# dbolya/yolact

Hardware: AMD Instinct MI355X
Metric: images/sec (550x550, batch 8 per GPU), YOLACT yolact_resnet50 forward + Detect (Fast NMS) (higher is better)
Workload: dtype f32 (fp32 in / fp32 accumulate / fp32 out; 92 % of the GEMM time on fp16x2 tiles = every fp32 operand as two fp16 pieces by round to nearest (22 significant bits + 2 signs: exact for ~2/3 of all fp32 values, one fp32 ulp otherwise), 3 exact piece products per product on the fp16 matrix pipe; measure

## Files before the change

### include/yolact_amd.h

```cpp
#ifndef YOLACT_AMD_H
#define YOLACT_AMD_H
#include <stddef.h>
#include <stdint.h>

#ifdef __cplusplus
extern "C" {
#endif

#define YMI_ABI_VERSION 9

#define YMI_EFORMAT (-4)
#define YMI_EUNSUPPORTED (-5)

enum { YMI_ACT_NONE = 0, YMI_ACT_RELU = 1, YMI_ACT_LEAKY01 = 2, YMI_ACT_TANH = 3, YMI_ACT_SIGMOID = 4 };
enum { YMI_RES_NONE = 0, YMI_RES_ADD = 1, YMI_RES_BILINEAR = 2 };

typedef struct {
  int32_t n0, n1;
  int32_t act;
  int32_t row_stride;
  int64_t batch_stride;
  float *ptr;
} ymi_conv_seg;

// ... 468 lines not shown
  const float *x;
  float *y;
  int32_t B, H, W, cout_pad;
  const void *w_h2;
  const float *scale_h2, *bias;
  float *y_amax;
  int32_t kpad, _pad0;
} ymi_stem_desc;
int ymi_stem_pool_f32(const ymi_stem_desc *d, void *stream);

typedef struct ymi_chain_desc {
  const float *x, *res;
  float *y, *z;
  const void *w_a_h2, *w_b_h2;
  const float *scale_a_h2, *bias_a, *scale_b_h2, *bias_b;
  const float *x_amax;
  float *y_amax, *z_amax;
  int64_t M;
  int32_t ldx, res_ld, ldy, ldz;
  int32_t k_a, n_a, n_b;
  int32_t cout_pad_a, cout_pad_b;
  int32_t act_a, act_b, _pad0;
  const float *res_amax;
  float gain_a, bias_max_a;
} ymi_chain_desc;
int ymi_pointwise_chain_f32(const ymi_chain_desc *d, void *stream);

typedef struct ymi_stage_exit_desc {
  ymi_chain_desc chain;
  int32_t B, H, W, y_stride;
} ymi_stage_exit_desc;
int ymi_stage_exit_chain_f32(const ymi_stage_exit_desc *d, void *stream);

enum { YMI_OP_NOP = 0, YMI_OP_CONV = 1, YMI_OP_WINO = 2, YMI_OP_DCN = 3, YMI_OP_CHAIN = 4, YMI_OP_STEM = 5, YMI_OP_INPUT = 6,
       YMI_OP_BILINEAR = 7, YMI_OP_MAXPOOL = 8, YMI_OP_BILINEAR_ADD = 9, YMI_OP_RECORD = 10, YMI_OP_WAIT = 11, YMI_OP_MEMSET = 12,
       YMI_OP_STAGE_EXIT = 13 };
enum { YMI_SEC_NONE = 0, YMI_SEC_BACKBONE = 1, YMI_SEC_FPN = 2, YMI_SEC_PROTO = 3, YMI_SEC_HEADS = 4 };
typedef struct ymi_plan_op {
  int32_t kind;
  int32_t stream;
  int32_t section;
  int32_t _pad;
  const void *desc;
  void *p[3];
  int64_t i[8];
  double f[2];
} ymi_plan_op;
int ymi_event_create(void **ev);
int ymi_event_destroy(void *ev);
int ymi_plan_run(const ymi_plan_op *ops, int first, int last, void *stream_a, void *stream_b, void *const *events, int overlap,
                 int skip_sections, int32_t *failed_op);

enum {
  YMI_WS_WINO_V = 1,
  YMI_WS_WINO_M = 2,
  YMI_WS_SPLITK = 3,
  YMI_WS_MASK_IOU = 4,
  YMI_WS_JPEG_COEFS = 5,
  YMI_WS_JPEG_PLANES = 6,
  YMI_WS_DETECT_SCORES_T = 7,
  YMI_WS_DETECT_PER_PRIOR = 8,
  YMI_WS_DETECT_CAND = 9,
  YMI_WS_DETECT_REC = 10,
  YMI_WS_AMAX_SLOT = 11,
  YMI_WS_RLE_COUNTS = 12,
  YMI_WS_DETECT_GREEDY = 13,
  YMI_WS_JPEG_ENC = 14,
  YMI_WS_JPEG_ENC_OUT = 15,
  YMI_WS_MASK_LOSS = 16,
// ... 31 lines not shown
```

### yolact_amd/_lib.py

```python
from __future__ import annotations

import ctypes as C
import os

_HERE = os.path.dirname(os.path.abspath(__file__))
LIB_PATH = os.path.join(_HERE, 'libyolact_amd.so')

ABI_VERSION = 9

ACT_NONE, ACT_RELU, ACT_LEAKY01, ACT_TANH, ACT_SIGMOID = 0, 1, 2, 3, 4
RES_NONE, RES_ADD, RES_BILINEAR = 0, 1, 2
TILE_AUTO, TILE_128x128, TILE_128x64, TILE_64x64, TILE_128x32, TILE_64x128 = 0, 1, 2, 3, 4, 5
TILE_32x32_K4, TILE_64x32_K2, TILE_32x64_K2 = 6, 7, 8
TILE_64x64_S3, TILE_64x64_S4, TILE_64x128_S3, TILE_128x64_S3, TILE_32x32_K4_S4, TILE_64x32_K2_S3, TILE_32x64_K2_S3 = range(9, 16)
TILE_NAMES = {1: '128x128', 2: '128x64', 3: '64x64', 4: '128x32', 5: '64x128', 6: '32x32k4', 7: '64x32k2', 8: '32x64k2',
              9: '64x64s3', 10: '64x64s4', 11: '64x128s3', 12: '128x64s3', 13: '32x32k4s4', 14: '64x32k2s3', 15: '32x64k2s3',
              16: '128x128w8', 17: '256x128w8', 18: '128x256w8', 19: '128x128s3', 20: '128x128w8s3', 21: '256x128w8s3',
              22: '128x128w8s4'}
TILE_128x128_W8, TILE_256x128_W8, TILE_128x256_W8 = 16, 17, 18
TILE_128x128_S3, TILE_128x128_W8_S3, TILE_256x128_W8_S3, TILE_128x128_W8_S4 = 19, 20, 21, 22
TILE_WG_128x256 = 23
TILE_X3 = 32
X3_BASE_TILES = (1, 2, 3, 5, 6, 7, 8, 9, 11, 12, 16, 17, 19, 20, 21, 22)
for _t in X3_BASE_TILES:
# ... 188 lines not shown


JPEG_SUB_444, JPEG_SUB_420 = 0, 2
JPEG_HEADER_BYTES = 623


class ChainDesc(C.Structure):
    _fields_ = [('x', C.c_void_p), ('res', C.c_void_p), ('y', C.c_void_p), ('z', C.c_void_p),
                ('w_a_h2', C.c_void_p), ('w_b_h2', C.c_void_p),
                ('scale_a_h2', C.c_void_p), ('bias_a', C.c_void_p), ('scale_b_h2', C.c_void_p), ('bias_b', C.c_void_p),
                ('x_amax', C.c_void_p), ('y_amax', C.c_void_p), ('z_amax', C.c_void_p),
                ('M', C.c_int64), ('ldx', C.c_int32), ('res_ld', C.c_int32), ('ldy', C.c_int32), ('ldz', C.c_int32),
                ('k_a', C.c_int32), ('n_a', C.c_int32), ('n_b', C.c_int32), ('cout_pad_a', C.c_int32), ('cout_pad_b', C.c_int32),
                ('act_a', C.c_int32), ('act_b', C.c_int32), ('_pad0', C.c_int32),
                ('res_amax', C.c_void_p), ('gain_a', C.c_float), ('bias_max_a', C.c_float)]


class StageExitDesc(C.Structure):
    _fields_ = [('chain', ChainDesc), ('B', C.c_int32), ('H', C.c_int32), ('W', C.c_int32), ('y_stride', C.c_int32)]


class StemDesc(C.Structure):
    _fields_ = [('x', C.c_void_p), ('y', C.c_void_p), ('B', C.c_int32), ('H', C.c_int32), ('W', C.c_int32), ('cout_pad', C.c_int32),
                ('w_h2', C.c_void_p), ('scale_h2', C.c_void_p), ('bias', C.c_void_p), ('y_amax', C.c_void_p),
                ('kpad', C.c_int32), ('_pad0', C.c_int32)]


class PlanOp(C.Structure):
    _fields_ = [('kind', C.c_int32), ('stream', C.c_int32), ('section', C.c_int32), ('_pad', C.c_int32), ('desc', C.c_void_p),
                ('p', C.c_void_p * 3), ('i', C.c_int64 * 8), ('f', C.c_double * 2)]


(OP_NOP, OP_CONV, OP_WINO, OP_DCN, OP_CHAIN, OP_STEM, OP_INPUT, OP_BILINEAR, OP_MAXPOOL, OP_BILINEAR_ADD, OP_RECORD, OP_WAIT,
 OP_MEMSET, OP_STAGE_EXIT) = range(14)
SEC_NONE, SEC_BACKBONE, SEC_FPN, SEC_PROTO, SEC_HEADS = range(5)


class MaskIouShape(C.Structure):
    _fields_ = [('A', C.c_int32), ('B', C.c_int32), ('n', C.c_int64)]


class ApMatchDesc(C.Structure):
    _fields_ = [('cls', C.c_void_p), ('box_score', C.c_void_p), ('mask_score', C.c_void_p), ('box_iou', C.c_void_p),
                ('mask_iou', C.c_void_p), ('crowd_box_iou', C.c_void_p), ('crowd_mask_iou', C.c_void_p), ('gt_cls', C.c_void_p),
                ('crowd_cls', C.c_void_p), ('rec_key', C.c_void_p), ('rec_score', C.c_void_p), ('rec_flags', C.c_void_p),
                ('gt_count', C.c_void_p), ('base', C.c_int64), ('cap', C.c_int64),
                ('N', C.c_int32), ('G', C.c_int32), ('Gc', C.c_int32), ('num_classes', C.c_int32)]


class ApFinalizeDesc(C.Structure):
    _fields_ = [('sorted_key', C.c_void_p), ('perm', C.c_void_p), ('rec_flags', C.c_void_p), ('gt_count', C.c_void_p),
                ('ap', C.c_void_p), ('empty', C.c_void_p), ('M', C.c_int64), ('cap', C.c_int64),
                ('num_classes', C.c_int32), ('_pad0', C.c_int32)]


AP_NUM_THRESH, AP_MAX_DET, AP_MAX_GT = 10, 1024, 2048


class RleShape(C.Structure):
    _fields_ = [('N', C.c_int32), ('h', C.c_int32), ('w', C.c_int32), ('cap', C.c_int32)]


(WS_WINO_V, WS_WINO_M, WS_SPLITK, WS_MASK_IOU, WS_JPEG_COEFS, WS_JPEG_PLANES, WS_DETECT_SCORES_T, WS_DETECT_PER_PRIOR,
 WS_DETECT_CAND, WS_DETECT_REC, WS_AMAX_SLOT, WS_RLE_COUNTS, WS_DETECT_GREEDY, WS_JPEG_ENC, WS_JPEG_ENC_OUT,
 WS_MASK_LOSS, WS_MATCH, WS_BOX_LOSS, WS_CLASS_LOSS, WS_SEGM_LOSS, WS_MASKIOU_INPUT, WS_CONV_BWD, WS_MASKIOU_HEAD,
 WS_CONV_WGRAD, WS_BN, WS_STEM_WGRAD) = range(1, 27)

# ... 29 lines not shown
    ('ymi_dcn_v2_forward_f32', C.c_int, [C.POINTER(DcnDesc), _P]),
    ('ymi_dcn_v2_backward_f32', C.c_int, [C.POINTER(DcnBwdDesc), _P]),
    ('ymi_mask_loss_f32', C.c_int, [C.POINTER(MaskLossDesc), _P]),
    ('ymi_match_f32', C.c_int, [C.POINTER(MatchDesc), _P]),
    ('ymi_box_loss_f32', C.c_int, [_P, _P, _P, _I, _I, _F, _P, _P, _P, _P]),
    ('ymi_class_loss_f32', C.c_int, [C.POINTER(ClassLossDesc), _P]),
    ('ymi_segm_loss_f32', C.c_int, [C.POINTER(SegmLossDesc), _P]),
    ('ymi_maskiou_input_f32', C.c_int, [C.POINTER(MaskIouInputDesc), _P]),
    ('ymi_maskiou_input_bwd_f32', C.c_int, [C.POINTER(MaskIouInputDesc), _P]),
    ('ymi_conv2d_bwd_nhwc_f32', C.c_int, [C.POINTER(ConvBwdDesc), _P]),
    ('ymi_global_maxpool_bwd_nhwc_f32', C.c_int, [_P, _P, _P, _I, _I, _I, _P]),
    ('ymi_maskiou_head_f32', C.c_int, [C.POINTER(MaskIouHeadDesc), _P]),
    ('ymi_act_bwd_f32', C.c_int, [_P, _P, _P, C.c_long] + [_I] * 6 + [_P]),
    ('ymi_conv_wgrad_nhwc_f32', C.c_int, [C.POINTER(ConvWgradDesc), _P]),
    ('ymi_conv_dgrad_s2_nhwc_f32', C.c_int, [C.POINTER(ConvDgradDesc), _P]),
    ('ymi_bn_fwd_nhwc_f32', C.c_int, [C.POINTER(BnDesc), _P]),
    ('ymi_bn_bwd_nhwc_f32', C.c_int, [C.POINTER(BnDesc), _P]),
    ('ymi_stem_wgrad_nhwc_f32', C.c_int, [C.POINTER(StemWgradDesc), _P]),
    ('ymi_maxpool_fwd_nhwc_f32', C.c_int, [_P, _P, _I, _I, _I, _I, _P]),
    ('ymi_maxpool_bwd_nhwc_f32', C.c_int, [_P, _P, _P, _I, _I, _I, _I, _P]),
    ('ymi_bilinear_bwd_nhwc_f32', C.c_int, [_P, _P, _P] + [_I] * 7 + [_P]),
    ('ymi_bilinear_size_bwd_nhwc_f32', C.c_int, [_P, _P] + [_I] * 6 + [_P]),
    ('ymi_composite_masks_u8', C.c_int, [_P, _P, _P, _I, _I, _I, _F, _P, _P]),
    ('ymi_mask_iou_f32', C.c_int, [_P, _P, _I, _I, C.c_long, _I, _P, _P, _P]),
    ('ymi_jaccard_f32', C.c_int, [_P, _P, _I, _I, _I, _P, _P]),
    ('ymi_mask_bits_f32', C.c_int, [_P, _I, C.c_long, _P, _P]),
    ('ymi_mask_upsample_bits', C.c_int, [_P, _I, _I, _I, _I, _I, _F, _P, _P]),
    ('ymi_mask_iou_bits', C.c_int, [_P, _P, _I, _I, C.c_long, _I, _P, _P]),
    ('ymi_ap_match_f32', C.c_int, [C.POINTER(ApMatchDesc), _P]),
    ('ymi_ap_finalize_f64', C.c_int, [C.POINTER(ApFinalizeDesc), _P]),
    ('ymi_stem_pool_f32', C.c_int, [_P, _P]),
    ('ymi_pointwise_chain_f32', C.c_int, [_P, _P]),
    ('ymi_stage_exit_chain_f32', C.c_int, [_P, _P]),
    ('ymi_mask_rle_f32', C.c_int, [_P, _I, _I, _I, _P, _P, _I, _P]),
    ('ymi_mask_rle_upsampled_f32', C.c_int, [_P, _I, _I, _I, _I, _I, _F, _P, _P, _I, _P]),
    ('ymi_rle_to_string', C.c_int, [_P, _P, _I, _I, _P, _P, _I, _P]),
    ('ymi_fast_base_transform_f32', C.c_int, [_P, _P, _I, _I, _I, _I, _I, C.POINTER(C.c_float), C.POINTER(C.c_float), _I, _I, _P]),
    ('ymi_jpeg_parse', C.c_int, [_P, C.c_size_t, C.POINTER(JpegInfo)]),
    ('ymi_jpeg_decode_coefs', C.c_int, [_P, C.c_size_t, _P, C.c_int64, _P, C.POINTER(JpegInfo)]),
    ('ymi_jpeg_reconstruct_bgr_u8', C.c_int, [C.POINTER(JpegInfo), _P, _P, _P, _P, _P]),
    ('ymi_jpeg_write_header', C.c_int, [_I, _I, _I, _I, _P, C.c_size_t, C.POINTER(C.c_size_t)]),
    ('ymi_jpeg_enc_qtables', C.c_int, [_I, _P]),
    ('ymi_jpeg_encode_bgr_u8', C.c_int, [C.POINTER(JpegEncDesc), _P]),
    ('ymi_coco_poly_fill_u8', C.c_int, [_P, _I, _I, _I, _P]),
    ('ymi_coco_rle_fill_u8', C.c_int, [_P, C.c_long, _I, _I, _P]),
    ('ymi_coco_rle_string_fill_u8', C.c_int, [C.c_char_p, C.c_long, _I, _I, _P]),
    ('ymi_event_create', C.c_int, [C.POINTER(C.c_void_p)]),
    ('ymi_event_destroy', C.c_int, [_P]),
    ('ymi_plan_run', C.c_int, [C.POINTER(PlanOp), _I, _I, _P, _P, C.POINTER(C.c_void_p), _I, _I, C.POINTER(C.c_int32)]),
    ('ymi_workspace_bytes', C.c_int64, [_I, _P]),
    ('ymi_calib_mfma_f16', C.c_int, [_P, _I, _I, C.POINTER(C.c_double), _P]),
    ('ymi_calib_hbm_copy', C.c_int, [_P, _P, C.c_long, C.POINTER(C.c_double), _P]),
    ('ymi_calib_l2_read', C.c_int, [_P, C.c_long, _I, _I, _P, C.POINTER(C.c_double), _P]),
    ('ymi_calib_latency', C.c_int, [_P, C.c_long, _I, _I, _P, _P]),
    ('ymi_debug_set_trace', C.c_int, [_P, C.c_long]),
    ('ymi_prof_enable', C.c_int, [_I]),
    ('ymi_prof_count', C.c_int, []),
    ('ymi_prof_read', C.c_int, [_I, C.POINTER(C.c_float), C.POINTER(C.c_double), C.POINTER(C.c_int32),
                                C.POINTER(C.c_int32)]),
    ('ymi_prof_reset', C.c_int, []),
]

_lib = None


def lib():
# ... 33 lines not shown
```

### yolact_amd/csrc/api.cpp

```cpp
#include "../../include/yolact_amd.h"
#include <hip/hip_runtime_api.h>

extern "C" {

int64_t ymi_detect_greedy_layout(const ymi_detect_desc *d, int64_t off[4]);
int64_t ymi_jpeg_enc_layout(int h, int w, int sub, int64_t off[8], int64_t *out_bound);
int64_t ymi_mask_loss_ws_bytes(const ymi_mask_loss_desc *d);
int64_t ymi_match_ws_bytes(const ymi_match_desc *d);
int64_t ymi_box_loss_ws_bytes(const ymi_match_desc *d);
int64_t ymi_class_loss_ws_bytes(const ymi_class_loss_desc *d);
int64_t ymi_segm_loss_ws_bytes(const ymi_segm_loss_desc *d);
int64_t ymi_maskiou_input_ws_bytes(const ymi_maskiou_input_desc *d);
int64_t ymi_conv_bwd_ws_bytes(const ymi_conv_bwd_desc *d);
int64_t ymi_maskiou_head_ws_bytes(const ymi_maskiou_head_desc *d);
int64_t ymi_conv_wgrad_ws_bytes(const ymi_conv_wgrad_desc *d);
int64_t ymi_bn_ws_bytes(const ymi_bn_desc *d);
int64_t ymi_stem_wgrad_ws_bytes(const ymi_stem_wgrad_desc *d);

int ymi_abi_version(void) { return YMI_ABI_VERSION; }

const char *ymi_strerror(int code) {
  switch (code) {
    case 0: return "ok";
    case -1: return "bad argument / unsupported configuration";
    case -2: return "shape or alignment constraint violated";
    case -3: return "null pointer";
    case YMI_EFORMAT: return "corrupt or truncated input stream";
    case YMI_EUNSUPPORTED: return "valid input outside the supported subset";
  }
  if (code > 0) return hipGetErrorString((hipError_t)code);
  return "unknown error";
}

int64_t ymi_workspace_bytes(int what, const void *desc) {
  auto cdiv = [](int64_t a, int64_t b) { return (a + b - 1) / b; };
  if (what == YMI_WS_AMAX_SLOT) return (int64_t)YMI_AMAX_SUB * YMI_AMAX_STRIDE * 4;
  if (!desc) return -3;
  switch (what) {
    case YMI_WS_WINO_V:
    case YMI_WS_WINO_M: {
      const ymi_wino_desc *d = (const ymi_wino_desc *)desc;
      const int m = d->m == 4 ? 4 : 2;
      if ((d->m != 0 && d->m != 2 && d->m != 4) || d->B < 1 || d->H < 1 || d->W < 1 || d->C < 1 || d->Cout < 1) return -1;
      const int64_t G = (int64_t)(m + 2) * (m + 2), T = (int64_t)d->B * cdiv(d->H, m) * cdiv(d->W, m);
      return 4 * G * T * (what == YMI_WS_WINO_V ? (int64_t)d->C : cdiv(d->Cout, 4) * 4);
    }
    case YMI_WS_SPLITK: {
      const ymi_conv_desc *d = (const ymi_conv_desc *)desc;
      if (d->B < 1 || d->Ho < 1 || d->Wo < 1 || d->Cout < 1 || d->split_k < 0) return -1;
      return d->split_k > 1 ? 4 * (int64_t)d->split_k * d->B * d->Ho * d->Wo * d->Cout : 0;
    }
    case YMI_WS_MASK_IOU: {
// ... 54 lines not shown
```

### yolact_amd/csrc/plan_exec.cpp

```cpp
#include "../../include/yolact_amd.h"
#include <hip/hip_runtime_api.h>

extern "C" {

int ymi_event_create(void **ev) {
  if (!ev) return -3;
  hipEvent_t e;
  const hipError_t rc = hipEventCreateWithFlags(&e, hipEventDisableTiming);
  if (rc != hipSuccess) return (int)rc;
  *ev = (void *)e;
  return 0;
}

int ymi_event_destroy(void *ev) {
  if (!ev) return -3;
  return (int)hipEventDestroy((hipEvent_t)ev);
}

int ymi_plan_run(const ymi_plan_op *ops, int first, int last, void *stream_a, void *stream_b, void *const *events, int overlap,
                 int skip_sections, int32_t *failed_op) {
  if (!ops || first < 0 || last < first) return -1;
  void *const sb = overlap ? stream_b : stream_a;
  for (int k = first; k < last; ++k) {
    const ymi_plan_op &o = ops[k];
    if (o.section && (skip_sections & (1 << o.section))) continue;
    void *const s = o.stream == 1 ? sb : stream_a;
    int rc = 0;
    switch (o.kind) {
      case YMI_OP_NOP: break;
      case YMI_OP_CONV: rc = ymi_conv2d_nhwc_f32((const ymi_conv_desc *)o.desc, s); break;
      case YMI_OP_WINO: rc = ymi_conv3x3_winograd_f32((const ymi_wino_desc *)o.desc, s); break;
      case YMI_OP_DCN: rc = ymi_dcn_v2_forward_f32((const ymi_dcn_desc *)o.desc, s); break;
      case YMI_OP_CHAIN: rc = ymi_pointwise_chain_f32((const ymi_chain_desc *)o.desc, s); break;
      case YMI_OP_STAGE_EXIT: rc = ymi_stage_exit_chain_f32((const ymi_stage_exit_desc *)o.desc, s); break;
      case YMI_OP_STEM: rc = ymi_stem_pool_f32((const ymi_stem_desc *)o.desc, s); break;
      case YMI_OP_INPUT:
        rc = o.p[2] ? ymi_nchw_to_nhwc4_amax_f32((const float *)o.p[0], (float *)o.p[1], (int)o.i[0], (int)o.i[1], (int)o.i[2], (int)o.i[3],
                                                 (float *)o.p[2], s)
                    : ymi_nchw_to_nhwc4_f32((const float *)o.p[0], (float *)o.p[1], (int)o.i[0], (int)o.i[1], (int)o.i[2], (int)o.i[3], s);
        break;
      case YMI_OP_BILINEAR:
        rc = ymi_bilinear_nhwc_f32((const float *)o.p[0], (float *)o.p[1], (int)o.i[0], (int)o.i[1], (int)o.i[2], (int)o.i[3], (int)o.i[4],
                                   (int)o.i[5], (float)o.f[0], (float)o.f[1], (int)o.i[6], s);
        break;
      case YMI_OP_MAXPOOL:
        rc = ymi_maxpool3x3s2_nhwc_f32((const float *)o.p[0], (float *)o.p[1], (int)o.i[0], (int)o.i[1], (int)o.i[2], (int)o.i[3],
                                       (int)o.i[4], (int)o.i[5], s);
        break;
      case YMI_OP_BILINEAR_ADD:
        rc = ymi_bilinear_add_nhwc_f32((const float *)o.p[0], (float *)o.p[1], (int)o.i[0], (int)o.i[1], (int)o.i[2], (int)o.i[3],
                                       (int)o.i[4], (int)o.i[5], (float *)o.p[2], s);
        break;
      case YMI_OP_RECORD:
        if (overlap) rc = (int)hipEventRecord((hipEvent_t)events[o.i[0]], (hipStream_t)s);
        break;
      case YMI_OP_WAIT:
        if (overlap) rc = (int)hipStreamWaitEvent((hipStream_t)s, (hipEvent_t)events[o.i[0]], 0);
        break;
      case YMI_OP_MEMSET:
        rc = (int)hipMemsetAsync(o.p[0], 0, (size_t)o.i[0], (hipStream_t)s);
        break;
      default: rc = -1;
    }
    if (rc != 0) {
      if (failed_op) *failed_op = k;
      return rc;
    }
// ... 6 lines not shown
```

### yolact_amd/engine.py

```python
from __future__ import annotations

import ctypes as C
import json
import os
from typing import List, Optional

import torch
import torch.nn as nn

from . import _lib as L
from .config import act_name, make_priors_host
from . import modules as M


def _ceil(a, b):
    return (a + b - 1) // b * b


SPLIT_DEFAULT = '2'
TUNE_GEN = 5
AMAX_SLOT_FLOATS = 16 * 64
TUNE_DIR = os.path.join(os.path.dirname(os.path.abspath(__file__)), 'tune')
_table_cache = {}

# ... 1074 lines not shown
        if timer is not None and not all(hasattr(timer, a) for a in ('start', 'stop', 'env')):
            timer = None
        if timer is None and self.native_exec:
            nat = self._native_plan()
            if nat is not None:
                det = self._run_native(nat, x, sa, sb, two, detect, skip_proto)
                self.mark_done()
                return proto, det
        if self.h2:
            self.amax[:self._nslots * AMAX_SLOT_FLOATS].zero_()
        self._sec = None
        try:
            det = self._dispatch(x, cur, sa, sb, two, detect, timer, skip_proto)
        finally:
            if timer is not None and self._sec is not None:
                timer.stop(self._sec)
        self.mark_done()
        return proto, det

    _SEC_ID = {'backbone': L.SEC_BACKBONE, 'fpn': L.SEC_FPN, 'proto': L.SEC_PROTO, 'pred_heads': L.SEC_HEADS}

    def _native_plan(self):
        key = (self.ops.version, len(self.ops)) if isinstance(self.ops, _OpList) else tuple(map(id, self.ops))
        if self._native is not None and self._native[0] == key:
            return self._native[1]
        lib = self.lib
        n = len(self.ops)
        arr = (L.PlanOp * (n + 1))()
        arr[0].kind, arr[0].stream = L.OP_MEMSET, 0
        arr[0].p[0], arr[0].i[0] = self.amax.data_ptr(), 4 * self._nslots * AMAX_SLOT_FLOATS
        ev_index, det_idx, in_idx, ok = {}, None, None, True
        by_fn = {id(lib.ymi_conv2d_nhwc_f32): L.OP_CONV, id(lib.ymi_conv3x3_winograd_f32): L.OP_WINO,
                 id(lib.ymi_dcn_v2_forward_f32): L.OP_DCN, id(lib.ymi_pointwise_chain_f32): L.OP_CHAIN,
                 id(lib.ymi_stage_exit_chain_f32): L.OP_STAGE_EXIT}
        for k, (fn, args, name, where) in enumerate(self.ops):
            o = arr[k + 1]
            o.stream = 1 if where == 'B' else 0
            o.section = self._SEC_ID.get(self.sections[k], 0) if self.sections[k] else 0
            if fn == 'input':
                a = self.in_args
                o.kind, in_idx = L.OP_INPUT, k + 1
                o.p[1] = a[1]
                o.p[2] = self.in_amax[2] if self.h2 else None
                o.i[0], o.i[1], o.i[2], o.i[3] = a[2], a[3], a[4], a[5]
            elif fn == 'stem':
                o.kind, o.desc = L.OP_STEM, C.addressof(args)
            elif fn == 'nop':
                o.kind = L.OP_NOP
            elif fn in ('record', 'wait'):
                o.kind = L.OP_RECORD if fn == 'record' else L.OP_WAIT
                o.i[0] = ev_index.setdefault(args, len(ev_index))
            elif fn == 'detect':
                o.kind, det_idx = L.OP_NOP, k + 1
            elif id(fn) in by_fn:
                o.kind, o.desc = by_fn[id(fn)], C.addressof(args.contents)
            elif fn is lib.ymi_bilinear_nhwc_f32:
                o.kind = L.OP_BILINEAR
                o.p[0], o.p[1] = args[0], args[1]
                for q in range(6):
                    o.i[q] = args[2 + q]
                o.f[0], o.f[1], o.i[6] = args[8].value, args[9].value, args[10]
            elif fn is lib.ymi_maxpool3x3s2_nhwc_f32:
                o.kind = L.OP_MAXPOOL
                o.p[0], o.p[1] = args[0], args[1]
                for q in range(6):
                    o.i[q] = args[2 + q]
            elif fn is lib.ymi_bilinear_add_nhwc_f32:
# ... 69 lines not shown
                a = self.in_args
                if self.h2:
                    rc = lib.ymi_nchw_to_nhwc4_amax_f32(x.data_ptr(), a[1], a[2], a[3], a[4], a[5], self.in_amax[2], s)
                else:
                    rc = lib.ymi_nchw_to_nhwc4_f32(x.data_ptr(), a[1], a[2], a[3], a[4], a[5], s)
            elif fn == 'nop' or (skip_proto and nsec == 'proto'):
                continue
            elif fn == 'stem':
                args.x = x.data_ptr()
                rc = lib.ymi_stem_pool_f32(C.byref(args), s)
            elif fn == 'record':
                if two:
                    self.events[args].record(self.stream_b if where == 'B' else cur)
                continue
            elif fn == 'wait':
                if two:
                    (self.stream_b if where == 'B' else cur).wait_event(self.events[args])
                continue
            elif fn == 'detect':
                if detect is not None:
                    det = detect(s)
                continue
            elif isinstance(args, tuple):
                rc = fn(*args, s)
            else:
                rc = fn(args, s)
            if rc != 0:
                L.check(rc, name)
        return det

    def tune(self, x: torch.Tensor, reps: int = 3):
        mode = os.environ.get('YOLACT_AMD_AUTOTUNE', '1')
        self.tune_table, self.wino_table, self.tune_misses = [], [], 0
        if mode == '0':
            return []
        cache_path = os.environ.get('YOLACT_AMD_TUNE_CACHE')
        disk = {}
        if mode != 'force':
            disk.update(load_tune_table(self.device))
            if cache_path and os.path.exists(cache_path):
                disk.update(_read_table_file(cache_path))
        n0 = len(disk)
        self.run(x)
        s = L.stream_ptr()
        e0, e1 = torch.cuda.Event(enable_timing=True), torch.cuda.Event(enable_timing=True)
        measure = mode != 'table'
        self._tune_direct(e0, e1, s, reps, disk, measure)
        self._tune_winograd(e0, e1, s, reps, disk, measure)
        self._fuse_pointwise_chains(e0, e1, s, reps, disk, measure)
        torch.cuda.synchronize(self.device)
        if cache_path and (len(disk) != n0 or mode == 'force'):
            _write_table_file(cache_path, disk, self.device)
        self.tune_entries = disk
        return self.tune_table

    autotune = tune

    def _splitk_ws(self, where, numel):
        ws = self._sk_ws.get(where)
        if ws is None or ws.numel() < numel:
            ws = self._sk_ws[where] = torch.empty(numel, dtype=torch.float32, device=self.device)
            for fn, dptr, _n, w in self.ops:
                if fn is self.lib.ymi_conv2d_nhwc_f32 and w == where and dptr.contents.split_k > 1:
                    dptr.contents.split_ws = ws.data_ptr()
                elif fn is self.lib.ymi_dcn_v2_forward_f32 and w == where and dptr.contents.conv.split_k > 1:
                    dptr.contents.conv.split_ws = ws.data_ptr()
        return ws

    @staticmethod
    def _splitk_ok(d):
        return (d.kh == 1 and d.kw == 1 and d.pad == 0 and d.Cin == d.Kpad and d.Cin % 32 == 0 and d.nseg == 1
                and d.Cout % 4 == 0 and d.seg[0].act <= L.ACT_LEAKY01 and d.res_mode in (L.RES_NONE, L.RES_ADD)
                and d.B * d.Ho * d.Wo <= 16384 and d.Kpad >= 256)

    def _fuse_pointwise_chains(self, e0, e1, s, reps, disk, measure):
        self.chain_table, self.chainx_table = [], []
        if not self.h2 or os.environ.get('YOLACT_AMD_CHAIN', '1') != '1':
            return
        lib = self.lib

        def timed(run):
            run()
# ... 168 lines not shown
            if overlap(zs, span(cd.y, cd.ldy)) or overlap(zs, span(cd.x, cd.ldx)) or (cd.res and overlap(zs, span(cd.res, cd.res_ld))):
                continue
            xptr = C.pointer(xd)
            name = n3 + '+' + n1
            shape = str((d3.B, d3.Ho, d3.Wo)) + self.mode_key
            ent = disk.get('chainx' + shape)
            if mode == 'force':
                ent = [1, 0.0, 0.0]
            if ent is None:
                self.tune_misses += 1
                if not measure or lib.ymi_stage_exit_chain_f32(xptr, s) != 0:
                    continue
                run3 = lambda: f3(p3, s)
                c1 = disk.get('chain1' + shape)
                if c1 is not None and c1[0]:
                    cc = L.ChainDesc.from_buffer_copy(cd)
                    cc.z, cc.w_b_h2, cc.scale_b_h2, cc.bias_b, cc.z_amax, cc.n_b = None, None, None, None, None, 64
                    ccp = C.pointer(cc)
                    if lib.ymi_pointwise_chain_f32(ccp, s) == 0:
                        run3 = lambda: lib.ymi_pointwise_chain_f32(ccp, s)
                t_plan = timed(lambda: (run3(), f1(p1, s)))
                t_one = timed(lambda: lib.ymi_stage_exit_chain_f32(xptr, s))
                ent = disk['chainx' + shape] = [1 if t_one < 0.97 * t_plan else 0, round(t_plan, 4), round(t_one, 4)]
            self.chainx_table.append((name, ent[0], ent[1], ent[2]))
            if ent[0] and lib.ymi_stage_exit_chain_f32(xptr, s) == 0:
                self.keepalive.append(xd)
                self.ops[i3] = (lib.ymi_stage_exit_chain_f32, xptr, name, w3)
                self.ops[i1] = ('nop', None, n1 + '[fused into ' + n3 + ']', w1)
                names = [n for n, _ in self.conv_meta]
                if n3 in names and n1 in names:
                    a, b = names.index(n3), names.index(n1)
                    if b > a + 1:
                        self.conv_meta.insert(a + 1, self.conv_meta.pop(b))

    def _apply_choice(self, fn, dptr, where, val, s):
        d = dptr.contents.conv if fn is self.lib.ymi_dcn_v2_forward_f32 else dptr.contents
        tile, S = int(val) & 255, int(val) >> 8
        d.tile = tile
        if S > 1:
            is_dcn = fn is self.lib.ymi_dcn_v2_forward_f32
            if tile & L.TILE_DCNP:
                nk_ = d.Kpad // 32
                if -(-nk_ // S) * (S - 1) >= nk_:
                    return -1
            elif is_dcn or not self._splitk_ok(d) or (d.Kpad // 32) % S:
                return -1
            d.split_k = S
            d.split_ws = self._splitk_ws(where, S * d.B * d.Ho * d.Wo * d.Cout).data_ptr()
        else:
            d.split_k = 0
        return fn(dptr, s)

    @staticmethod
    def _pipe_ok(d):
        return ((d.kh, d.kw, d.pad) in ((3, 3, 1), (1, 1, 0)) and d.Cin % 32 == 0 and d.Kpad == d.kh * d.kw * d.Cin and d.Kpad >= 64
                and d.nseg == 1 and d.Cout % 4 == 0 and d.seg[0].n0 == 0 and d.seg[0].act <= L.ACT_LEAKY01
                and d.seg[0].row_stride % 4 == 0 and d.seg[0].batch_stride == d.Ho * d.Wo * d.seg[0].row_stride
                and d.res_mode in (L.RES_NONE, L.RES_ADD))

    @staticmethod
    def dcnp_candidates(d, dcn=False):
        M, nk = d.B * d.Ho * d.Wo, d.Kpad // 32
        out = []
        for t, name in sorted(L.DCNP_TILES.items()):
            bm, bn = (int(v) for v in name[4:].split('w')[0].split('x'))
            if (bn > 128 and d.Cout < 256) or (dcn and t in L.DCNP_PLAIN_ONLY) or (bn == 32) != (d.Cout <= 32):
# ... 274 lines not shown
```

Baseline: 2362.

## Add specialized persistent kernel for 1x1 expand convs with autotuned install

Adds a dedicated persistent HIP kernel for 1x1 stride-1 expansion convolutions (Cin 128/256, Cout = 4*Cin). Each block keeps its 256-wide weight slice in registers, streams activation rows through a register ring, and splits them to fp16 hi/lo pieces in LDS for the three-product MFMA scheme, with a fused scale/bias/activation/residual epilogue. The kernel is timed against the existing conv path during autotuning and installed only when it wins by a margin. This adds a new kernel, a plan op kind and tuning-cache entries, and relies on grid sizing by CU count and on specific shape constraints.

```diff
diff --git a/include/yolact_amd.h b/include/yolact_amd.h
--- a/include/yolact_amd.h
+++ b/include/yolact_amd.h
@@ -524,9 +524,11 @@
 } ymi_stage_exit_desc;
 int ymi_stage_exit_chain_f32(const ymi_stage_exit_desc *d, void *stream);
 
+int ymi_conv1x1_expand_f32(const ymi_conv_desc *d, void *stream);
+
 enum { YMI_OP_NOP = 0, YMI_OP_CONV = 1, YMI_OP_WINO = 2, YMI_OP_DCN = 3, YMI_OP_CHAIN = 4, YMI_OP_STEM = 5, YMI_OP_INPUT = 6,
        YMI_OP_BILINEAR = 7, YMI_OP_MAXPOOL = 8, YMI_OP_BILINEAR_ADD = 9, YMI_OP_RECORD = 10, YMI_OP_WAIT = 11, YMI_OP_MEMSET = 12,
-       YMI_OP_STAGE_EXIT = 13 };
+       YMI_OP_STAGE_EXIT = 13, YMI_OP_EXPAND = 14 };
 enum { YMI_SEC_NONE = 0, YMI_SEC_BACKBONE = 1, YMI_SEC_FPN = 2, YMI_SEC_PROTO = 3, YMI_SEC_HEADS = 4 };
 typedef struct ymi_plan_op {
   int32_t kind;
diff --git a/yolact_amd/_lib.py b/yolact_amd/_lib.py
--- a/yolact_amd/_lib.py
+++ b/yolact_amd/_lib.py
@@ -244,7 +244,7 @@
 
 
 (OP_NOP, OP_CONV, OP_WINO, OP_DCN, OP_CHAIN, OP_STEM, OP_INPUT, OP_BILINEAR, OP_MAXPOOL, OP_BILINEAR_ADD, OP_RECORD, OP_WAIT,
- OP_MEMSET, OP_STAGE_EXIT) = range(14)
+ OP_MEMSET, OP_STAGE_EXIT, OP_EXPAND) = range(15)
 SEC_NONE, SEC_BACKBONE, SEC_FPN, SEC_PROTO, SEC_HEADS = range(5)
 
 
@@ -340,6 +340,7 @@
     ('ymi_stem_pool_f32', C.c_int, [_P, _P]),
     ('ymi_pointwise_chain_f32', C.c_int, [_P, _P]),
     ('ymi_stage_exit_chain_f32', C.c_int, [_P, _P]),
+    ('ymi_conv1x1_expand_f32', C.c_int, [C.POINTER(ConvDesc), _P]),
     ('ymi_mask_rle_f32', C.c_int, [_P, _I, _I, _I, _P, _P, _I, _P]),
     ('ymi_mask_rle_upsampled_f32', C.c_int, [_P, _I, _I, _I, _I, _I, _F, _P, _P, _I, _P]),
     ('ymi_rle_to_string', C.c_int, [_P, _P, _I, _I, _P, _P, _I, _P]),
diff --git a/yolact_amd/csrc/api.cpp b/yolact_amd/csrc/api.cpp
--- a/yolact_amd/csrc/api.cpp
+++ b/yolact_amd/csrc/api.cpp
@@ -1,5 +1,7 @@
 #include "../../include/yolact_amd.h"
 #include <hip/hip_runtime_api.h>
+
+int ymi_internal_expand_conv(const ymi_conv_desc *d, hipStream_t s);
 
 extern "C" {
 
@@ -18,6 +20,11 @@
 int64_t ymi_stem_wgrad_ws_bytes(const ymi_stem_wgrad_desc *d);
 
 int ymi_abi_version(void) { return YMI_ABI_VERSION; }
+
+int ymi_conv1x1_expand_f32(const ymi_conv_desc *d, void *stream) {
+  if (!d) return -3;
+  return ymi_internal_expand_conv(d, (hipStream_t)stream);
+}
 
 const char *ymi_strerror(int code) {
   switch (code) {
diff --git a/yolact_amd/csrc/expand.hip b/yolact_amd/csrc/expand.hip
--- /dev/null
+++ b/yolact_amd/csrc/expand.hip
@@ -0,0 +1,258 @@
+#include "gemm_h2.h"
+#include <stdlib.h>
+#include <type_traits>
+
+int ymi_internal_prof_begin(double flops, int tile, int kind, hipStream_t s);
+void ymi_internal_prof_end(int idx, hipStream_t s);
+
+namespace {
+
+using namespace ymi_h2;
+
+typedef unsigned u32x4 __attribute__((ext_vector_type(4)));
+
+constexpr int BM = 64, BN = 256, NWAVE = 8, NT = 64 * NWAVE;
+constexpr int A_BYTES = 2 * BM * 64, B_BYTES = 2 * BN * 64;
+constexpr int NSA = 3, NSU = 3;
+constexpr int JT = BM / 32, NU = 4 * JT;
+constexpr int RA = BM / (NT / 8);
+constexpr int OFF_SC = NSA * A_BYTES, OFF_BI = OFF_SC + BN * 4, OFF_U = OFF_BI + BN * 4, EX_LDS = OFF_U + NSU * B_BYTES;
+constexpr int UPC = (2 * BN / 16) / NWAVE;
+static_assert(UPC == 4 && RA == 1 && JT == 2 && EX_LDS <= 160 * 1024, "block shape");
+#define EX_PIN() __builtin_amdgcn_sched_barrier(0)
+#define EX_MFMA(a, b, c) __builtin_amdgcn_mfma_f32_32x32x16_f16(a, b, c, 0, 0, 0)
+
+struct ExParams {
+  const float *x, *scale_h2, *bias, *x_amax, *res;
+  const void *w_h2;
+  float *y, *y_amax;
+  int M, ldx, Cout, cout_pad, ldy, res_ld, res_after_act, act;
+  int tiles_n, bpc, groups;
+  unsigned w_plane;
+};
+
+template <int NK>
+__global__ __launch_bounds__(NT) void expand_us_k(const ExParams p) {
+#if defined(__HIP_DEVICE_COMPILE__)
+  __shared__ __attribute__((aligned(16))) char lds[EX_LDS];
+  const int t = threadIdx.x, lane = t & 63, wave = __builtin_amdgcn_readfirstlane(t >> 6);
+  const int lr = lane & 31, hh = lane >> 5;
+  const int lb = ymi_xcd_remap((int)blockIdx.x, (int)gridDim.x);
+  const int tn = lb / p.bpc, jb = lb % p.bpc;
+  const int row0 = 32 * (int)(((long)jb * p.groups) / p.bpc);
+  int rend = 32 * (int)(((long)(jb + 1) * p.groups) / p.bpc);
+  rend = rend < p.M ? rend : p.M;
+  const int ntile = (rend - row0 + BM - 1) / BM;
+
+  const bool has_res = p.res != nullptr;
+  const __amdgpu_buffer_rsrc_t xrs = buf_rsrc(p.x, rend * p.ldx * 4);
+  const __amdgpu_buffer_rsrc_t wrs = buf_rsrc(p.w_h2, 2 * p.w_plane);
+  const __amdgpu_buffer_rsrc_t rrs = buf_rsrc(p.res, has_res ? rend * p.res_ld * 4 : 0);
+  const __amdgpu_buffer_rsrc_t yrs = buf_rsrc(p.y, rend * p.ldy * 4);
+  const ymi_amax_pre apre = ymi_amax_prefetch(p.y_amax);
+
+  const int kq = t & 7, r0 = t >> 3;
+  const int a_st = r0 * 64 + (((kq >> 1) ^ ((r0 >> 2) & 3)) * 16) + (kq & 1) * 8;
+  unsigned a_vo = (unsigned)((row0 + r0) * p.ldx + 4 * kq) * 4u;
+  f32x4 ring[2][RA];
+  static_assert(NK >= 4 && NK % 2 == 0, "the ring runs four chunks ahead of the MFMAs");
+  auto request = [&](int S, int kc) {
+    const unsigned vo = kc < NK ? a_vo : a_vo + (unsigned)(BM * p.ldx) * 4u;
+    const int kk = kc < NK ? kc : kc - NK;
+#pragma unroll
+    for (int i = 0; i < RA; ++i)
+      ring[S][i] = __builtin_bit_cast(f32x4, __builtin_amdgcn_raw_buffer_load_b128(xrs, vo + (unsigned)(64 * i * p.ldx) * 4u, kk * (BK * 4), 0));
+  };
+  float sA, invA;
+  auto wait_vm = [](int n) {
+    switch (n) {
+#define EX_W(v) case v: YMI_WAIT_VM(v); break;
+      EX_W(1) EX_W(2) EX_W(3) EX_W(4) EX_W(5) EX_W(6) EX_W(7) EX_W(8) EX_W(9) EX_W(10) EX_W(11) EX_W(12) EX_W(13) EX_W(14) EX_W(15) EX_W(16)
+      EX_W(17) EX_W(18) EX_W(19) EX_W(20) EX_W(21) EX_W(22) EX_W(23) EX_W(24) EX_W(25) EX_W(26) EX_W(27) EX_W(28)
+#undef EX_W
+      default: YMI_WAIT_VM(0);
+    }
+  };
+  auto combine = [&](int S, int stage) {
+#pragma unroll
+    for (int i = 0; i < RA; ++i) {
+      f16x4 h4, l4;
+      split4h(ring[S][i], sA, h4, l4);
+      char *dst = lds + stage * A_BYTES + a_st + i * 4096;
+      *reinterpret_cast<f16x4 *>(dst) = h4;
+      *reinterpret_cast<f16x4 *>(dst + BM * 64) = l4;
+    }
+  };
+  int b_dst[UPC];
+  unsigned b_vo[UPC];
+#pragma unroll
+  for (int i = 0; i < UPC; ++i) {
+    const int q = wave + NWAVE * i, plane = q >> 4, rg = q & 15;
+    const int row = rg * 16 + (lane >> 2), lsl = (lane & 3) ^ ((row >> 2) & 3), grow = tn * BN + row;
+    b_dst[i] = plane * (BN * 64) + rg * 1024;
+    b_vo[i] = grow < p.cout_pad ? (unsigned)plane * p.w_plane + 16u * lsl + (unsigned)(grow * (NK * BK)) * 2u : OOB;
+  }
+  auto upieces = [&](int kc) {
+#pragma unroll
+    for (int i = 0; i < UPC; ++i)
+      __builtin_amdgcn_raw_ptr_buffer_load_lds(wrs, (lds_ptr_t)(lds + OFF_U + (kc % NSU) * B_BYTES + b_dst[i]), 16, b_vo[i], (unsigned)kc * 64u, 0, 0);
+  };
+
+  f16x8 u[2][2 * NK];
+  f32x16 acc[JT];
+#pragma unroll
+  for (int j = 0; j < JT; ++j)
+#pragma unroll
+    for (int r = 0; r < 16; ++r) acc[j][r] = 0.f;
+  const int psw = (lr >> 2) & 3;
+  const int fo[2] = {lr * 64 + 16 * ((0 + hh) ^ psw), lr * 64 + 16 * ((2 + hh) ^ psw)};
+  const float *sc = reinterpret_cast<const float *>(lds + OFF_SC) + 32 * wave + 4 * hh;
+  const float *bi = reinterpret_cast<const float *>(lds + OFF_BI) + 32 * wave + 4 * hh;
+  const float slope = ymi_act_slope(p.act);
+  const int ncol = tn * BN + 32 * wave + 4 * hh;
+  float am = 0.f;
+
+  auto res_load = [&](int trow, int q) {
+    const int row = trow + 32 * (q >> 2) + lr, n = ncol + 8 * (q & 3);
+    return __builtin_bit_cast(f32x4, __builtin_amdgcn_raw_buffer_load_b128(rrs, n < p.Cout ? (unsigned)(row * p.res_ld + n) * 4u : OOB, 0, 0));
+  };
+  auto finish = [&](int trow, int q, const f32x4 rv) {
+    const int j = q >> 2, gq = q & 3;
+    const int row = trow + 32 * j + lr, n = ncol + 8 * gq;
+    const f32x4 s4 = *reinterpret_cast<const f32x4 *>(sc + 8 * gq), b4 = *reinterpret_cast<const f32x4 *>(bi + 8 * gq);
+    f32x4 v;
+#pragma unroll
+    for (int e = 0; e < 4; ++e) { v[e] = acc[j][4 * gq + e]; acc[j][4 * gq + e] = 0.f; }
+    v = v * s4 + b4;
+    if (has_res && !p.res_after_act) v += rv;
+#pragma unroll
+    for (int e = 0; e < 4; ++e) v[e] = fmaxf(v[e], slope * v[e]);
+    if (has_res && p.res_after_act) v += rv;
+    if (row < rend && n < p.Cout) am = fmaxf(am, ymi_absmax4(v));
+    __builtin_amdgcn_raw_buffer_store_b128(__builtin_bit_cast(u32x4, v), yrs, n < p.Cout ? (unsigned)(row * p.ldy + n) * 4u : OOB, 0, 0);
+  };
+
+  f32x4 rv[NU];
+  request(0, 0);
+  upieces(0);
+  request(1, 1);
+  upieces(1);
+  EX_PIN();
+  ymi_h2_scale(ymi_amax_read(p.x_amax), sA, invA);
+  if (t < 64) {
+    const int n = tn * BN + 4 * t;
+    f32x4 s4 = {0.f, 0.f, 0.f, 0.f}, b4 = {0.f, 0.f, 0.f, 0.f};
+    if (n < p.Cout) {
+      s4 = *reinterpret_cast<const f32x4 *>(p.scale_h2 + n);
+      if (p.bias) b4 = *reinterpret_cast<const f32x4 *>(p.bias + n);
+    }
+    *reinterpret_cast<f32x4 *>(lds + OFF_SC + 16 * t) = s4 * invA;
+    *reinterpret_cast<f32x4 *>(lds + OFF_BI + 16 * t) = b4;
+  }
+  combine(0, 0);
+  combine(1, 1);
+  request(0, 2);
+  request(1, 3);
+  EX_PIN();
+#pragma unroll
+  for (int q = 0; q < NU; ++q) rv[q] = res_load(row0, q);
+  EX_PIN();
+  wait_vm(2 * RA + NU);
+  YMI_BARRIER();
+
+  int st = 0;
+  auto tile = [&](auto first_, int trow) {
+    constexpr bool FIRST = decltype(first_)::value;
+    const bool both = trow + 32 < rend;
+#pragma unroll
+    for (int kc = 0; kc < NK; ++kc) {
+      const int sn = st == NSA - 1 ? 0 : st + 1, sn2 = st == 0 ? NSA - 1 : st - 1;
+      if constexpr (FIRST) {
+        const char *ub = lds + OFF_U + (kc % NSU) * B_BYTES + (32 * wave) * 64;
+#pragma unroll
+        for (int pl = 0; pl < 2; ++pl)
+#pragma unroll
+          for (int s2 = 0; s2 < 2; ++s2) u[pl][2 * kc + s2] = *reinterpret_cast<const f16x8 *>(ub + pl * (BN * 64) + fo[s2]);
+      }
+      const bool ureq = FIRST && kc + 2 < NK;
+      if (ureq) upieces(kc + 2);
+      if (kc == 0 && !FIRST) {
+#pragma unroll
+        for (int q = 0; q < NU; ++q) rv[q] = res_load(trow, q);
+      }
+      const char *ab = lds + st * A_BYTES;
+#pragma unroll
+      for (int s2 = 0; s2 < 2; ++s2) {
+        EX_PIN();
+        const f16x8 ah0 = *reinterpret_cast<const f16x8 *>(ab + fo[s2]), al0 = *reinterpret_cast<const f16x8 *>(ab + fo[s2] + BM * 64);
+        if (s2 == 0) {
+          combine(kc & 1, sn2);
+          request(kc & 1, kc + 4);
+        }
+        if (both) {
+          const f16x8 ah1 = *reinterpret_cast<const f16x8 *>(ab + fo[s2] + 2048), al1 = *reinterpret_cast<const f16x8 *>(ab + fo[s2] + 2048 + BM * 64);
+#pragma unroll
+          for (int pr = 0; pr < 3; ++pr) {
+            acc[0] = EX_MFMA(u[pr == 0 ? 1 : 0][2 * kc + s2], pr == 1 ? al0 : ah0, acc[0]);
+            acc[1] = EX_MFMA(u[pr == 0 ? 1 : 0][2 * kc + s2], pr == 1 ? al1 : ah1, acc[1]);
+          }
+        } else {
+#pragma unroll
+          for (int pr = 0; pr < 3; ++pr) acc[0] = EX_MFMA(u[pr == 0 ? 1 : 0][2 * kc + s2], pr == 1 ? al0 : ah0, acc[0]);
+        }
+      }
+      st = sn;
+      EX_PIN();
+      if (FIRST && kc >= 1 && kc + 1 < NK) wait_vm(RA + (ureq ? UPC : 0) + RA);
+      YMI_BARRIER();
+    }
+#pragma unroll
+    for (int q = 0; q < NU; ++q) finish(trow, q, rv[q]);
+    a_vo += (unsigned)(BM * p.ldx) * 4u;
+  };
+  tile(std::true_type{}, row0);
+  for (int k = 1; k < ntile; ++k) tile(std::false_type{}, row0 + k * BM);
+  if (p.y_amax) ymi_amax_finish(apre, am);
+#endif
+}
+
+}
+
+int ymi_internal_expand_conv(const ymi_conv_desc *d, hipStream_t s) {
+  const ymi_conv_seg &g0 = d->seg[0];
+  if (d->kh != 1 || d->kw != 1 || d->stride != 1 || d->pad != 0 || d->nseg != 1 || d->split_k > 1) return YMI_EARG;
+  if ((d->Cin != 128 && d->Cin != 256) || d->Kpad != d->Cin || d->ldx < d->Cin || (d->Cout & 3) || d->Cout < 4) return YMI_EARG;
+  if (d->Ho != d->H || d->Wo != d->W || d->B < 1 || d->H < 1 || d->W < 1) return YMI_EARG;
+  if (d->res_mode != YMI_RES_NONE && d->res_mode != YMI_RES_ADD) return YMI_EARG;
+  if (g0.n0 != 0 || g0.n1 < d->Cout || g0.act > YMI_ACT_LEAKY01 || g0.act < 0) return YMI_EARG;
+  if (!d->x || !g0.ptr || !d->w_h2 || !d->scale_h2 || !d->x_amax || (d->res_mode == YMI_RES_ADD && !d->res)) return YMI_ENULL;
+  const long HW = (long)d->H * d->W, M = (long)d->B * HW;
+  if ((d->ldx & 3) || (g0.row_stride & 3) || g0.row_stride < d->Cout || g0.batch_stride != HW * g0.row_stride) return YMI_ESHAPE;
+  if ((((uintptr_t)d->x) | ((uintptr_t)g0.ptr) | ((uintptr_t)d->w_h2) | ((uintptr_t)d->scale_h2) | ((uintptr_t)d->bias)) & 15) return YMI_ESHAPE;
+  if (d->res_mode == YMI_RES_ADD && ((d->res_ld & 3) || d->res_ld < d->Cout || (((uintptr_t)d->res) & 15))) return YMI_ESHAPE;
+  if ((M + 256) * d->ldx * 4 >= (1L << 31) || M * g0.row_stride * 4 >= (1L << 31) || (d->res_mode == YMI_RES_ADD && M * d->res_ld * 4 >= (1L << 31)))
+    return YMI_ESHAPE;
+  ExParams p;
+  p.x = d->x; p.scale_h2 = d->scale_h2; p.bias = d->bias; p.x_amax = d->x_amax; p.w_h2 = d->w_h2;
+  p.res = d->res_mode == YMI_RES_ADD ? d->res : nullptr;
+  p.y = g0.ptr; p.y_amax = d->y_amax;
+  p.M = (int)M; p.ldx = d->ldx; p.Cout = d->Cout; p.cout_pad = (d->Cout + 127) / 128 * 128; p.ldy = g0.row_stride;
+  p.res_ld = d->res_ld; p.res_after_act = d->res_after_act; p.act = g0.act;
+  p.w_plane = (unsigned)((long)p.cout_pad * d->Kpad * 2L);
+  int dev = 0, cus = 256;
+  hipGetDevice(&dev);
+  hipDeviceGetAttribute(&cus, hipDeviceAttributeMultiprocessorCount, dev);
+  { const char *e = getenv("YMI_EXPAND_BLOCKS"); if (e && atoi(e) > 0) cus = atoi(e); }
+  const int tiles_m = (int)((M + BM - 1) / BM);
+  p.tiles_n = (d->Cout + BN - 1) / BN;
+  p.groups = (int)((M + 31) / 32);
+  p.bpc = cus / p.tiles_n < 1 ? 1 : (cus / p.tiles_n < tiles_m ? cus / p.tiles_n : tiles_m);
+  const dim3 grid((unsigned)(p.tiles_n * p.bpc));
+  const double flops = 2.0 * (double)M * (double)(d->cout_alg > 0 ? d->cout_alg : d->Cout) * (double)(d->cin_alg > 0 ? d->cin_alg : d->Cin);
+  const int pr = ymi_internal_prof_begin(flops, d->tile, 10, s);
+  if (d->Cin == 256) hipLaunchKernelGGL(expand_us_k<8>, grid, dim3(NT), 0, s, p);
+  else hipLaunchKernelGGL(expand_us_k<4>, grid, dim3(NT), 0, s, p);
+  const int rc = ymi_launch_status();
+  ymi_internal_prof_end(pr, s);
+  return rc;
+}
diff --git a/yolact_amd/csrc/plan_exec.cpp b/yolact_amd/csrc/plan_exec.cpp
--- a/yolact_amd/csrc/plan_exec.cpp
+++ b/yolact_amd/csrc/plan_exec.cpp
@@ -33,6 +33,7 @@
       case YMI_OP_DCN: rc = ymi_dcn_v2_forward_f32((const ymi_dcn_desc *)o.desc, s); break;
       case YMI_OP_CHAIN: rc = ymi_pointwise_chain_f32((const ymi_chain_desc *)o.desc, s); break;
       case YMI_OP_STAGE_EXIT: rc = ymi_stage_exit_chain_f32((const ymi_stage_exit_desc *)o.desc, s); break;
+      case YMI_OP_EXPAND: rc = ymi_conv1x1_expand_f32((const ymi_conv_desc *)o.desc, s); break;
       case YMI_OP_STEM: rc = ymi_stem_pool_f32((const ymi_stem_desc *)o.desc, s); break;
       case YMI_OP_INPUT:
         rc = o.p[2] ? ymi_nchw_to_nhwc4_amax_f32((const float *)o.p[0], (float *)o.p[1], (int)o.i[0], (int)o.i[1], (int)o.i[2], (int)o.i[3],
diff --git a/yolact_amd/engine.py b/yolact_amd/engine.py
--- a/yolact_amd/engine.py
+++ b/yolact_amd/engine.py
@@ -1130,7 +1130,7 @@
         ev_index, det_idx, in_idx, ok = {}, None, None, True
         by_fn = {id(lib.ymi_conv2d_nhwc_f32): L.OP_CONV, id(lib.ymi_conv3x3_winograd_f32): L.OP_WINO,
                  id(lib.ymi_dcn_v2_forward_f32): L.OP_DCN, id(lib.ymi_pointwise_chain_f32): L.OP_CHAIN,
-                 id(lib.ymi_stage_exit_chain_f32): L.OP_STAGE_EXIT}
+                 id(lib.ymi_stage_exit_chain_f32): L.OP_STAGE_EXIT, id(lib.ymi_conv1x1_expand_f32): L.OP_EXPAND}
         for k, (fn, args, name, where) in enumerate(self.ops):
             o = arr[k + 1]
             o.stream = 1 if where == 'B' else 0
@@ -1266,6 +1266,9 @@
     def tune(self, x: torch.Tensor, reps: int = 3):
         mode = os.environ.get('YOLACT_AMD_AUTOTUNE', '1')
         self.tune_table, self.wino_table, self.tune_misses = [], [], 0
+        for i, (f, p, n, w) in enumerate(self.ops):
+            if not isinstance(f, str) and f is self.lib.ymi_conv1x1_expand_f32:
+                self.ops[i] = (self.lib.ymi_conv2d_nhwc_f32, p, n, w)
         if mode == '0':
             return []
         cache_path = os.environ.get('YOLACT_AMD_TUNE_CACHE')
@@ -1282,6 +1285,19 @@
         self._tune_direct(e0, e1, s, reps, disk, measure)
         self._tune_winograd(e0, e1, s, reps, disk, measure)
         self._fuse_pointwise_chains(e0, e1, s, reps, disk, measure)
+
+        def timed(run):
+            run()
+            best = 1e30
+            for _ in range(2):
+                e0.record()
+                for _ in range(reps):
+                    run()
+                e1.record()
+                e1.synchronize()
+                best = min(best, e0.elapsed_time(e1) / reps)
+            return best
+        self._install_expand(s, disk, measure, timed)
         torch.cuda.synchronize(self.device)
         if cache_path and (len(disk) != n0 or mode == 'force'):
             _write_table_file(cache_path, disk, self.device)
@@ -1516,6 +1532,48 @@
                     a, b = names.index(n3), names.index(n1)
                     if b > a + 1:
                         self.conv_meta.insert(a + 1, self.conv_meta.pop(b))
+
+    def expand_candidates(self):
+        conv = self.lib.ymi_conv2d_nhwc_f32
+        out = []
+        for i, (f, p, _n, _w) in enumerate(self.ops):
+            if f is not conv or i in self.wide_ops:
+                continue
+            d = p.contents
+            if ((d.kh, d.kw, d.stride, d.pad, d.nseg) == (1, 1, 1, 0, 1) and d.Cin in (128, 256) and d.Cout == 4 * d.Cin
+                    and d.Kpad == d.Cin and d.ldx >= d.Cin and (d.Ho, d.Wo) == (d.H, d.W) and d.split_k <= 1
+                    and d.res_mode in (L.RES_NONE, L.RES_ADD) and d.seg[0].n0 == 0 and d.seg[0].act <= L.ACT_LEAKY01
+                    and d.seg[0].row_stride % 4 == 0 and d.seg[0].batch_stride == d.Ho * d.Wo * d.seg[0].row_stride):
+                out.append(i)
+        return out
+
+    def _install_expand(self, s, disk, measure, timed=None, launch=True):
+        mode = os.environ.get('YOLACT_AMD_EXPAND', '1')
+        self.expand_table = []
+        lib = self.lib
+        if not self.h2 or mode not in ('1', 'force'):
+            return
+        for i in self.expand_candidates():
+            f, p, n, w = self.ops[i]
+            d = p.contents
+            if launch:
+                base = d.tile & 31
+                if not (d.w_h2 and d.x_amax and (d.tile & L.TILE_DCNP) and (d.tile & L.TILE_H2) and 1 <= base <= 19):
+                    continue
+            key = 'expand' + str((d.B, d.Ho, d.Wo, d.Cin, d.Cout)) + self.mode_key
+            ent = disk.get(key)
+            if mode == 'force':
+                ent = [1, 0.0, 0.0]
+            if ent is None:
+                self.tune_misses += 1
+                if not (measure and launch and timed is not None) or lib.ymi_conv1x1_expand_f32(p, s) != 0:
+                    continue
+                t_pipe = timed(lambda: f(p, s))
+                t_exp = timed(lambda: lib.ymi_conv1x1_expand_f32(p, s))
+                ent = disk[key] = [1 if t_exp < 0.97 * t_pipe else 0, round(t_pipe, 4), round(t_exp, 4)]
+            self.expand_table.append((n, ent[0], ent[1], ent[2]))
+            if ent[0] and (not launch or lib.ymi_conv1x1_expand_f32(p, s) == 0):
+                self.ops[i] = (lib.ymi_conv1x1_expand_f32, p, n, w)
 
     def _apply_choice(self, fn, dptr, where, val, s):
         d = dptr.contents.conv if fn is self.lib.ymi_dcn_v2_forward_f32 else dptr.contents
```

Result: no change. 2355 (-0.3%).
